# nicrie/xmca

Measured on AMD Instinct MI355X. Metric: MCA solve+rotate throughput (ms_per_step = solve+rotate wall-clock, ms); rule_n surrogates/s in `rule_n`, higher is better.
Workload: dtype f64; 1 GPU; C2: synthetic EOF T=2920 x N=10000 float64 (generator A), solve() + rotate(n_rot=10, power=1); parallelism=replicas x1 (solve/rotate do not shard); rule_n run-sharded x1

## Files before the change

xmca_amd/build.py:

```python
import os
import shutil
import subprocess
import sys

HERE = os.path.dirname(os.path.abspath(__file__))
CSRC = os.path.join(HERE, "csrc")
REPO = os.path.dirname(HERE)
LIB = os.path.join(HERE, "libxmca_hip.so")
SOURCES = ["xmca_hip.cpp"]
HEADERS = ["chol64.h", "cholesky.h", "comm.h", "common.h", "fft.h", "gemm.h", "jacobi.h", "jacobi_kernels.h", "kernels.h", "rotate.h", "solver.h", "theta.h", "tridiag.h", "tridiag_vec.h"]
ARCH = "gfx950"


def _hipcc():
    for cand in (os.environ.get("HIPCC"), shutil.which("hipcc"), "/opt/rocm/bin/hipcc"):
        if cand and os.path.exists(cand):
            return cand
    raise RuntimeError("hipcc not found (set HIPCC)")


def needs_build():
    if not os.path.exists(LIB):
        return True
    t = os.path.getmtime(LIB)
    deps = [os.path.join(CSRC, f) for f in SOURCES + HEADERS] + [os.path.join(REPO, "include", "xmca_hip.h")]
    return any(os.path.getmtime(d) > t for d in deps)


def build(force=False, verbose=True):
    if not force and not needs_build():
        return LIB
    cmd = [_hipcc(), "-x", "hip", "--offload-arch=" + ARCH, "-O3", "-std=c++17", "-fPIC", "-shared",
           "-Wall", "-Wno-unused-function", "-Wno-unused-variable", "-Wno-unused-but-set-variable",
           "-I", os.path.join(REPO, "include")]
    cmd += os.environ.get("XMCA_EXTRA_CXXFLAGS", "").split()
    cmd += [os.path.join(CSRC, s) for s in SOURCES]
    cmd += ["-ldl", "-o", LIB + ".tmp"]
    if verbose:
        print(" ".join(cmd), flush=True)
    subprocess.run(cmd, check=True)
    os.replace(LIB + ".tmp", LIB)
    return LIB

# ... 5 lines not shown
```

xmca_amd/csrc/cholesky.h:

```cpp
#pragma once
#include <hip/hip_runtime.h>

#include <cmath>
#include <cstring>

#include "common.h"
#include "gemm.h"
#include "kernels.h"
#include "chol64.h"

namespace xmca {

constexpr int CHOL_NB = C64;

__global__ void chol_zero_lower_kernel(double* __restrict__ Gr, double* __restrict__ Gi, int64_t ld, int n, const double* __restrict__ Dr,
                                       const double* __restrict__ Di) {
  const int64_t total = (int64_t)n * n;
  for (int64_t i = (int64_t)blockIdx.x * blockDim.x + threadIdx.x; i < total; i += (int64_t)gridDim.x * blockDim.x) {
    const int r = (int)(i / n), c = (int)(i % n);
    if (r > c) {
      Gr[(int64_t)r * ld + c] = 0.0;
      if (Gi) Gi[(int64_t)r * ld + c] = 0.0;
    } else if ((r >> 6) == (c >> 6)) {
      const int64_t o = (int64_t)(r >> 6) * 4096 + (r & 63) * 64 + (c & 63);
// ... 3 lines not shown
  }
}

__global__ void chol_shift_diag_kernel(double* __restrict__ Gr, int64_t ld, int n, double delta) {
  const int i = blockIdx.x * blockDim.x + threadIdx.x;
  if (i < n) Gr[(int64_t)i * ld + i] += delta;
}

__global__ void chol_max_diag_kernel(const double* __restrict__ Gr, int64_t ld, int n, unsigned long long* __restrict__ out) {
  double mx = 0.0;
  for (int i = blockIdx.x * blockDim.x + threadIdx.x; i < n; i += gridDim.x * blockDim.x) mx = fmax(mx, Gr[(int64_t)i * ld + i]);
  for (int o = 32; o > 0; o >>= 1) mx = fmax(mx, __shfl_xor(mx, o));
  if ((threadIdx.x & 63) == 0 && mx > 0.0) atomicMax(out, (unsigned long long)__double_as_longlong(mx));
}

__global__ void chol_minmax_diag_kernel(const double* __restrict__ Gr, int64_t ld, int n, unsigned long long* __restrict__ out) {
  double mx = 0.0, mn = HUGE_VAL;
  for (int i = blockIdx.x * blockDim.x + threadIdx.x; i < n; i += gridDim.x * blockDim.x) {
    const double v = Gr[(int64_t)i * ld + i];
    mx = fmax(mx, v);
    mn = fmin(mn, v);
  }
  for (int o = 32; o > 0; o >>= 1) { mx = fmax(mx, __shfl_xor(mx, o)); mn = fmin(mn, __shfl_xor(mn, o)); }
  if ((threadIdx.x & 63) == 0) {
    if (mx > 0.0) atomicMax(out, (unsigned long long)__double_as_longlong(mx));
    if (mn >= 0.0) atomicMin(out + 1, (unsigned long long)__double_as_longlong(mn));
  }
}

template <typename TI>
void cgemm(hipStream_t st, GemmWorkspace& ws, const TI* Ar, const TI* Ai, int64_t lda, bool a_kfast, bool conjA, const TI* Br,
           const TI* Bi, int64_t ldb, bool b_nfast, bool conjB, double* Cr, double* Ci, int64_t ldc, int M, int N, int K,
           double alpha, const double* row_scale, const double* col_scale, bool herm, double beta0 = 0.0,
           const GemmTileList* tiles = nullptr, int plan_rows = 0) {
  GemmOpts o;
  o.tiles = tiles;
  o.plan_rows = plan_rows;
  o.a_kfast = a_kfast;
  o.b_nfast = b_nfast;
  o.row_scale = row_scale;
  o.col_scale = col_scale;
  o.upper_only = herm;
  const double sa = conjA ? -1.0 : 1.0, sb = conjB ? -1.0 : 1.0;
  o.alpha = alpha; o.beta = beta0; o.mirror = herm ? 1 : 0;
  gemm<TI, double>(st, ws, Ar, lda, Br, ldb, Cr, ldc, M, N, K, o);
  if (Ai && Bi) {
    o.alpha = -sa * sb * alpha; o.beta = 1.0;
    gemm<TI, double>(st, ws, Ai, lda, Bi, ldb, Cr, ldc, M, N, K, o);
  }
  if (!Ci) return;
  o.mirror = herm ? -1 : 0;
  bool first = true;
  if (Bi) {
    o.alpha = sb * alpha; o.beta = beta0;
    gemm<TI, double>(st, ws, Ar, lda, Bi, ldb, Ci, ldc, M, N, K, o);
    first = false;
  }
  if (Ai) {
    o.alpha = sa * alpha; o.beta = first ? beta0 : 1.0;
    gemm<TI, double>(st, ws, Ai, lda, Br, ldb, Ci, ldc, M, N, K, o);
    first = false;
  }
  if (first && beta0 == 0.0) XMCA_HIP(hipMemsetAsync(Ci, 0, sizeof(double) * (size_t)M * ldc, st));
}

template <bool CPLX>
static void chol64_launch_panel(hipStream_t st, double* Gr, double* Gi, int64_t ld, int k0, int nb, int rest, double* Dr, double* Di, int* fail) {
  XMCA_HIP(hipFuncSetAttribute(reinterpret_cast<const void*>(chol64_panel_kernel<CPLX>), hipFuncAttributeMaxDynamicSharedMemorySize, (int)C64Lds<CPLX>::bytes()));
// ... 56 lines not shown
```

xmca_amd/csrc/gemm.h:

```cpp
#pragma once
#include <algorithm>
#include <cmath>
#include <memory>
#include <type_traits>
#include <vector>

#include "common.h"

namespace xmca {

typedef double d4_t __attribute__((ext_vector_type(4)));
typedef float f4_t __attribute__((ext_vector_type(4)));
typedef double d2_t __attribute__((ext_vector_type(2)));
typedef float f2_t __attribute__((ext_vector_type(2)));

template <typename T>
struct Mfma;
template <>
struct Mfma<double> {
  using acc_t = d4_t;
  using vec_t = d2_t;
  using frag_t = d2_t;
  static __device__ __forceinline__ acc_t mma(double a, double b, acc_t c) {
    return __builtin_amdgcn_mfma_f64_16x16x4f64(a, b, c, 0, 0, 0);
  }
  static __device__ __forceinline__ int row(int lane, int r) { return (lane >> 4) + 4 * r; }
};
template <>
struct Mfma<float> {
  using acc_t = f4_t;
  using vec_t = f4_t;
  using frag_t = f2_t;
  static __device__ __forceinline__ acc_t mma(float a, float b, acc_t c) {
    return __builtin_amdgcn_mfma_f32_16x16x4f32(a, b, c, 0, 0, 0);
  }
  static __device__ __forceinline__ int row(int lane, int r) { return (lane >> 4) * 4 + r; }
};

constexpr int GEMM_BM = 128, GEMM_BN = 128, GEMM_THREADS = 256;
constexpr int GEMM_STAGE_BYTES = 16384;
constexpr int GEMM_FLUSH_PRODUCTS = 512;
constexpr int GEMM_SLICE_PRODUCTS = 16384;
template <typename T>
struct GemmK {
  static constexpr int E = (int)sizeof(T);
  static constexpr int CE = 16 / E;
  static constexpr int BK = 128 / E;
  static constexpr int NPH = BK / 8;
};

template <typename TI, typename TO>
struct GemmParams {
  const TI* A;
  const TI* B;
  TO* C;
  int M, N, K;
  int64_t lda, ldb, ldc;
  double alpha, beta;
  const double* row_scale;
  const double* col_scale;
  int upper_only;
  int mirror;
  int k_chunk;
  int splits;
  int n_tiles;
  int n_wg;
  const int* tile_map;
  const int* tile_k;
  int vec_a, vec_b;
  double* slabs;
  int* counters;
};

template <typename TI, bool KFAST>
struct GemmOperand {
  static constexpr int E = GemmK<TI>::E, CE = GemmK<TI>::CE, BK = GemmK<TI>::BK;
  using frag_t = typename Mfma<TI>::frag_t;
  static __device__ __forceinline__ void where(int o, int& r, int& k) {
    if constexpr (KFAST) {
      r = o >> 7;
      k = (((o >> 4) & 7) ^ ((r >> 1) & 7)) * CE;
    } else {
      k = o / (128 * E);
      int c = (o % (128 * E)) >> 4;
      if constexpr (E == 4) c ^= ((k >> 1) & 1) << 3;
      r = c * CE;
    }
  }
  static __device__ __forceinline__ uint32_t voff(int lane, int jpar, int64_t ld) {
    if constexpr (KFAST) return (uint32_t)((lane >> 3) * ld * E + (((lane & 7) ^ (((lane >> 4) + 4 * jpar) & 7)) << 4));
    else if constexpr (E == 8) return (uint32_t)(lane * 16);
    else return (uint32_t)((lane >> 5) * ld * E + (((lane & 31) ^ (jpar << 3)) << 4));
  }
  static __device__ __forceinline__ uint32_t soff(int wave, int j, int64_t ld) {
    const int q = 4 * wave + j;
    return (uint32_t)((KFAST ? 8 : (E == 8 ? 1 : 2)) * q * ld * E);
  }
  static __device__ __forceinline__ uint32_t remaining(int R, int row0, int K, int k0, int64_t ld) {
    const int64_t n = KFAST ? ((int64_t)(R - 1 - row0) * ld + (K - k0)) * E : ((int64_t)(K - 1 - k0) * ld + (R - row0)) * E;
    return n > 0xffffffffll ? 0xffffffffu : (uint32_t)n;
  }
  static __device__ __forceinline__ int frag_base(int w0, int lane) {
    const int i = lane & 15, kk = lane >> 4;
    if constexpr (KFAST) {
// ... 38 lines not shown
  l = h ^ m;
  return;
#endif
  const f2_t x[4] = {f2_t{x0[0], x0[1]}, f2_t{x0[2], x0[3]}, f2_t{x1[0], x1[1]}, f2_t{x1[2], x1[3]}};
#pragma unroll
  for (int q = 0; q < 4; ++q) {
    const unsigned int hp = __builtin_bit_cast(unsigned int, __builtin_convertvector(x[q], bf16x2_t));
    h[q] = hp;
    const f2_t r = x[q] - f2_t{__uint_as_float(hp << 16), __uint_as_float(hp & 0xffff0000u)};
    const unsigned int mp = __builtin_bit_cast(unsigned int, __builtin_convertvector(r, bf16x2_t));
    m[q] = mp;
    const f2_t t = r - f2_t{__uint_as_float(mp << 16), __uint_as_float(mp & 0xffff0000u)};
    l[q] = __builtin_bit_cast(unsigned int, __builtin_convertvector(t, bf16x2_t));
  }
}

template <typename TI, typename TO, bool A_KFAST, bool B_NFAST, bool WIDE, bool X3 = false>
__global__ __launch_bounds__(GEMM_THREADS, 2) void gemm_kernel(GemmParams<TI, TO> p) {
  static_assert(!X3 || (std::is_same<TI, float>::value && A_KFAST && WIDE), "X3: float32, A contiguous along the contraction");
  using M_ = Mfma<TI>;
  using acc_t = typename M_::acc_t;
  using vec_t = typename M_::vec_t;
  using frag_t = typename M_::frag_t;
  using OA = GemmOperand<TI, A_KFAST>;
  using OB = GemmOperand<TI, !B_NFAST>;
  constexpr int CE = GemmK<TI>::CE, BK = GemmK<TI>::BK, NPH = GemmK<TI>::NPH, E = GemmK<TI>::E, SB = GEMM_STAGE_BYTES;
  __shared__ __attribute__((aligned(1024))) char smem[4 * SB];

  int L;
  {
    const int b = blockIdx.x, q = p.n_wg / 8, r = p.n_wg % 8, xcd = b % 8, idx = b / 8;
    L = (xcd < r ? xcd * (q + 1) : r * (q + 1) + (xcd - r) * q) + idx;
  }
  const int split = L / p.n_tiles, tile = L % p.n_tiles;
  const int packed = p.tile_map[tile];
  const int bm = packed >> 16, bn = packed & 0xffff;
  const int bm0 = bm * GEMM_BM, bn0 = bn * GEMM_BN;
  int kbeg, kend;
  if (p.tile_k) {
    const int kb = p.tile_k[2 * tile], ke = p.tile_k[2 * tile + 1];
    const int kc = ((ke - kb + GemmK<TI>::BK * p.splits - 1) / (GemmK<TI>::BK * p.splits)) * GemmK<TI>::BK;
    kbeg = kb + split * kc;
    kend = max(kbeg, min(ke, kbeg + kc));
  } else {
    kbeg = split * p.k_chunk;
    kend = min(p.K, kbeg + p.k_chunk);
  }

  const int wave = __builtin_amdgcn_readfirstlane((int)threadIdx.x >> 6);
  int lane = gemm_lane_id();
  const int wm = (wave >> 1) * 64, wn = (wave & 1) * 64;

  acc_t acc[X3 ? 1 : 4][X3 ? 1 : 4];
  acc_t wide[(WIDE && !X3) ? 4 : 1][(WIDE && !X3) ? 4 : 1];
  f16v_t acc3[X3 ? 2 : 1][X3 ? 2 : 1], wide3[X3 ? 2 : 1][X3 ? 2 : 1];
  if constexpr (X3) {
#pragma unroll
    for (int i = 0; i < 2; ++i)
#pragma unroll
      for (int j = 0; j < 2; ++j)
#pragma unroll
        for (int g = 0; g < 16; ++g) { acc3[i][j][g] = 0.f; wide3[i][j][g] = 0.f; }
  } else {
#pragma unroll
    for (int i = 0; i < 4; ++i)
#pragma unroll
      for (int j = 0; j < 4; ++j) {
        acc[i][j] = acc_t{0, 0, 0, 0};
        if constexpr (WIDE) wide[i][j] = acc_t{0, 0, 0, 0};
      }
  }

  const char* tileA = reinterpret_cast<const char*>(A_KFAST ? p.A + (int64_t)bm0 * p.lda : p.A + bm0);
  const char* tileB = reinterpret_cast<const char*>(B_NFAST ? p.B + bn0 : p.B + (int64_t)bn0 * p.ldb);
  const int64_t kstepA = (A_KFAST ? 1 : p.lda) * E, kstepB = (B_NFAST ? p.ldb : 1) * E;
  uint32_t va[2], vb[2];
#pragma unroll
  for (int jp = 0; jp < 2; ++jp) {
    va[jp] = OA::voff(lane, jp, p.lda);
    vb[jp] = OB::voff(lane, jp, p.ldb);
// ... 186 lines not shown
  for (int kt = nfull; kt < nkt; ++kt) {
    __syncthreads();
    stage_slow(kbeg + kt * BK, 0, tid);
    __syncthreads();
    if constexpr (X3) {
#pragma unroll
      for (int q = 0; q < 2; ++q) {
        read_frags3(smem, q);
        split3();
        mma3();
      }
    } else {
#pragma unroll
      for (int q = 0; q < NPH; ++q) {
        read_frags(smem, q, af[0], bf[0]);
        mfmas(af[0], bf[0]);
      }
    }
    flush(kt);
  }

  d2_t tot[32];
#pragma unroll
  for (int r = 0; r < 64; ++r) {
    double v;
    if constexpr (X3) v = (double)acc3[r >> 5][(r >> 4) & 1][r & 15] + (double)wide3[r >> 5][(r >> 4) & 1][r & 15];
    else {
      v = (double)acc[r >> 4][(r >> 2) & 3][r & 3];
      if constexpr (WIDE) v += (double)wide[r >> 4][(r >> 2) & 3][r & 3];
    }
    tot[r >> 1][r & 1] = v;
  }

  if (p.splits > 1) {
    double* __restrict__ mine = p.slabs + ((size_t)split * p.n_tiles + tile) * (size_t)(GEMM_BM * GEMM_BN);
#if defined(__HIP_DEVICE_COMPILE__)
    {
      const __amdgpu_buffer_rsrc_t rs = __builtin_amdgcn_make_buffer_rsrc(mine, 0, GEMM_BM * GEMM_BN * 8, 0x00020000);
#pragma unroll
      for (int h = 0; h < 32; ++h)
        __builtin_amdgcn_raw_buffer_store_b128(__builtin_bit_cast(u4_t, tot[h]), rs, tid * 16, h * 4096,  16);
    }
#endif
    asm volatile("s_waitcnt vmcnt(0)" ::: "memory");
    __syncthreads();
    int* flag = reinterpret_cast<int*>(smem);
    if (tid == 0) {
      const int ticket = __hip_atomic_fetch_add(p.counters + tile, 1, __ATOMIC_RELAXED, __HIP_MEMORY_SCOPE_AGENT);
      const int last = ticket == p.splits - 1;
      if (last) {
        __builtin_amdgcn_fence(__ATOMIC_ACQUIRE, "agent");
        __hip_atomic_store(p.counters + tile, 0, __ATOMIC_RELAXED, __HIP_MEMORY_SCOPE_AGENT);
      }
      *flag = last;
    }
    __syncthreads();
    if (*flag == 0) return;
#pragma unroll
    for (int h = 0; h < 32; ++h) tot[h] = d2_t{0, 0};
    for (int z = 0; z < p.splits; ++z) {
      const d2_t* __restrict__ sl = reinterpret_cast<const d2_t*>(p.slabs + ((size_t)z * p.n_tiles + tile) * (size_t)(GEMM_BM * GEMM_BN));
#pragma unroll
      for (int h0 = 0; h0 < 32; h0 += 8) {
#pragma unroll
        for (int h = h0; h < h0 + 8; ++h) tot[h] += sl[h * GEMM_THREADS + tid];
        asm volatile("" ::: "memory");
      }
    }
  }

  const bool offdiag = (bm != bn);
  TO* __restrict__ C = p.C;
#pragma unroll
  for (int r = 0; r < 64; ++r) {
    int rin, cin;
    if constexpr (X3) {
      const int g = r & 15;
      rin = 32 * (r >> 5) + (g & 3) + 8 * (g >> 2) + 4 * (lane >> 5);
      cin = 32 * ((r >> 4) & 1) + (lane & 31);
    } else {
      rin = OA::index(r >> 4, M_::row(lane, r & 3));
      cin = OB::index((r >> 2) & 3, lane & 15);
    }
    const int row = bm0 + wm + rin, col = bn0 + wn + cin;
    const bool sym_diag = p.mirror > 0 && !offdiag;
    if (row < p.M && col < p.N && !(sym_diag && col < row)) {
      double v = tot[r >> 1][r & 1] * p.alpha;
      if (p.row_scale) v *= p.row_scale[row];
      if (p.col_scale) v *= p.col_scale[col];
      const int64_t o = (int64_t)row * p.ldc + col;
      if (p.beta != 0.0) v += p.beta * (double)C[o];
      C[o] = (TO)v;
      if ((p.mirror != 0 && offdiag) || (sym_diag && col > row)) C[(int64_t)col * p.ldc + row] = (TO)(p.mirror > 0 ? v : -v);
    }
  }
}

struct GemmTileList {
  DevBuf<int> map;
  DevBuf<int> krange;
  int n = 0;
  int klen = 0;
  void upload(hipStream_t st, const std::vector<int>& tiles, const std::vector<int>& kr) {
    n = (int)tiles.size();
    klen = 0;
    for (int t = 0; t < n; ++t) klen = std::max(klen, kr[2 * t + 1] - kr[2 * t]);
    if (n == 0) return;
    XMCA_HIP(hipMemcpyAsync(map.ensure(tiles.size()), tiles.data(), sizeof(int) * tiles.size(), hipMemcpyHostToDevice, st));
    XMCA_HIP(hipMemcpyAsync(krange.ensure(kr.size()), kr.data(), sizeof(int) * kr.size(), hipMemcpyHostToDevice, st));
    XMCA_HIP(hipStreamSynchronize(st));
  }
};

struct GemmOpts {
  bool a_kfast = true;
  bool b_nfast = true;
  double alpha = 1.0, beta = 0.0;
  const double* row_scale = nullptr;
  const double* col_scale = nullptr;
  bool upper_only = false;
  int mirror = 0;
  int force_splits = 0;
  int plan_rows = 0;
  const GemmTileList* tiles = nullptr;
  hipEvent_t ev_begin = nullptr, ev_end = nullptr;
};

struct GemmWorkspace {
  DevBuf<double> slabs;
  DevBuf<int> counters;
  size_t counters_ready = 0;
  struct Map { int tm, tn, upper; DevBuf<int> dev; int n; };
  std::vector<std::unique_ptr<Map>> maps;
  int n_cus = 0;

  const Map& tile_map(hipStream_t st, int tm, int tn, bool upper) {
    for (auto& m : maps)
      if (m->tm == tm && m->tn == tn && m->upper == (int)upper) return *m;
    constexpr int G = 8;
    std::vector<int> order;
    for (int si = 0; si < tm; si += G)
      for (int sj = upper ? si : 0; sj < tn; sj += G)
        for (int i = si; i < std::min(si + G, tm); ++i)
          for (int j = sj; j < std::min(sj + G, tn); ++j)
            if (!upper || j >= i) order.push_back((i << 16) | j);
    auto m = std::make_unique<Map>();
    m->tm = tm; m->tn = tn; m->upper = upper; m->n = (int)order.size();
    XMCA_HIP(hipMemcpyAsync(m->dev.ensure(order.size()), order.data(), sizeof(int) * order.size(), hipMemcpyHostToDevice, st));
    XMCA_HIP(hipStreamSynchronize(st));
    maps.push_back(std::move(m));
    return *maps.back();
  }
  int* tickets(hipStream_t st, size_t n) {
    if (n > counters_ready) {
      const size_t want = std::max<size_t>(n, 4096);
      int* c = counters.ensure(want);
      XMCA_HIP(hipMemsetAsync(c, 0, sizeof(int) * counters.cap, st));
      counters_ready = counters.cap;
    }
    return counters.get();
  }
  int cus() {
    if (n_cus == 0) {
      int dev = 0, n = 256;
      (void)hipGetDevice(&dev);
      (void)hipDeviceGetAttribute(&n, hipDeviceAttributeMultiprocessorCount, dev);
      n_cus = n > 0 ? n : 256;
    }
    return n_cus;
  }
};

static inline bool gemm_x3_enabled() {
  static const bool on = [] { const char* e = std::getenv("XMCA_GEMM_BF16X3"); return !(e && e[0] == '0'); }();
  return on;
}

template <typename TI, typename TO, bool WIDE>
static void launch_gemm_variant(hipStream_t st, const GemmParams<TI, TO>& p, bool a_kfast, bool b_nfast) {
  dim3 grid(p.n_wg), block(GEMM_THREADS);
  if constexpr (std::is_same<TI, float>::value) {
    if (a_kfast && gemm_x3_enabled()) {
      if (b_nfast) hipLaunchKernelGGL((gemm_kernel<TI, TO, true, true, WIDE, true>), grid, block, 0, st, p);
      else hipLaunchKernelGGL((gemm_kernel<TI, TO, true, false, WIDE, true>), grid, block, 0, st, p);
      XMCA_HIP(hipGetLastError());
      return;
    }
  }
  if (a_kfast && b_nfast) hipLaunchKernelGGL((gemm_kernel<TI, TO, true, true, WIDE>), grid, block, 0, st, p);
  else if (a_kfast && !b_nfast) hipLaunchKernelGGL((gemm_kernel<TI, TO, true, false, WIDE>), grid, block, 0, st, p);
  else if (!a_kfast && b_nfast) hipLaunchKernelGGL((gemm_kernel<TI, TO, false, true, WIDE>), grid, block, 0, st, p);
  else hipLaunchKernelGGL((gemm_kernel<TI, TO, false, false, WIDE>), grid, block, 0, st, p);
  XMCA_HIP(hipGetLastError());
}

static inline int gemm_choose_splits(int64_t tiles, int nkt, int n_cus) {
  const int max_s = std::min(std::max(nkt / 4, 1), 128);
  int best_s = 1;
  double best = 1e300;
  for (int s = 1; s <= max_s; ++s) {
    const double q = (double)tiles * s / (2.0 * n_cus);
    const double fl = std::floor(q), phi = q - fl;
    const double rounds = fl * 1.73 + (phi < 1e-9 ? 0.0 : (phi <= 0.5 ? 1.0 : 1.73));
    const double cost = ((double)nkt / s + 8.0) * rounds * (1.0 + 0.005 * s) + (s > 1 ? (double)s : 0.0);
    if (cost < best) { best = cost; best_s = s; }
  }
  return best_s;
}

template <typename TI, typename TO>
void gemm(hipStream_t st, GemmWorkspace& ws, const TI* A, int64_t lda, const TI* B, int64_t ldb, TO* C, int64_t ldc, int M,
          int N, int K, const GemmOpts& o) {
  if (M <= 0 || N <= 0) return;
  XMCA_CHECK(!o.upper_only || M == N, XMCA_ERR_INVALID, "gemm: upper_only needs a square result");
  constexpr int BK = GemmK<TI>::BK, CE = GemmK<TI>::CE;
  const int tm = ceil_div(M, GEMM_BM), tn = ceil_div(N, GEMM_BN);
  constexpr bool WIDE = std::is_same<TI, float>::value;
  const GemmTileList* list = o.tiles;
  XMCA_CHECK(!list || (!o.upper_only && o.mirror == 0 && !WIDE), XMCA_ERR_INVALID, "gemm: tile lists are plain float64 products");
  if (list && list->n == 0) return;
  const int64_t tiles = list ? list->n : o.upper_only ? (int64_t)tm * (tm + 1) / 2 : (int64_t)tm * tn;
  const int klen = list ? list->klen : K;
  const int nkt = ceil_div(klen, BK);
  const int64_t tiles_plan = (o.plan_rows > 0 && !list && !o.upper_only) ? (int64_t)ceil_div(o.plan_rows, GEMM_BM) * tn : tiles;
  int splits = o.force_splits > 0 ? o.force_splits : gemm_choose_splits(tiles_plan, nkt, ws.cus());
  if (WIDE) splits = std::max(splits, ceil_div(K, GEMM_SLICE_PRODUCTS));
  const int* map_dev = nullptr;
  if (list) {
    map_dev = list->map.get();
  } else {
    const GemmWorkspace::Map& map = ws.tile_map(st, tm, tn, o.upper_only);
    XMCA_CHECK(map.n == tiles && tm < 65536 && tn < 65536, XMCA_ERR_INVALID, "gemm: tile map mismatch");
    map_dev = map.dev.get();
  }
  const int vec_a = lda * (int64_t)sizeof(TI) * 128 < ((int64_t)1 << 32) && reinterpret_cast<uintptr_t>(A) % sizeof(TI) == 0;
  const int vec_b = ldb * (int64_t)sizeof(TI) * 128 < ((int64_t)1 << 32) && reinterpret_cast<uintptr_t>(B) % sizeof(TI) == 0;
  int k_chunk = klen > 0 ? klen : 1;
  if (splits > 1) {
    k_chunk = ceil_div(nkt, splits) * BK;
    if (WIDE) k_chunk = std::min(k_chunk, GEMM_SLICE_PRODUCTS);
    splits = ceil_div(klen, k_chunk);
  }
  if (splits < 1 || klen <= 0) splits = 1;
  XMCA_CHECK(tiles * splits < (int64_t)1 << 31, XMCA_ERR_INVALID, "gemm: too many workgroups");
  double* slabs = nullptr;
  int* counters = nullptr;
  if (splits > 1) {
    slabs = ws.slabs.ensure((size_t)splits * tiles * GEMM_BM * GEMM_BN);
    counters = ws.tickets(st, (size_t)tiles);
  }
  GemmParams<TI, TO> p{A, B, C, M, N, K, lda, ldb, ldc, o.alpha, o.beta, o.row_scale, o.col_scale, o.upper_only ? 1 : 0, o.mirror,
                       k_chunk, splits, (int)tiles, (int)(tiles * splits), map_dev, list ? list->krange.get() : nullptr, vec_a, vec_b,
                       slabs, counters};
  if (o.ev_begin) XMCA_HIP(hipEventRecord(o.ev_begin, st));
  launch_gemm_variant<TI, TO, WIDE>(st, p, o.a_kfast, o.b_nfast);
  if (o.ev_end) XMCA_HIP(hipEventRecord(o.ev_end, st));
}

}
```

xmca_amd/csrc/tridiag_vec.h:

```cpp
#pragma once
#include "cholesky.h"
#include "tridiag.h"

namespace xmca {

__device__ __forceinline__ double trd_lane_value(double v, int u) {
  const int lo = __builtin_amdgcn_readlane(__double2loint(v), u), hi = __builtin_amdgcn_readlane(__double2hiint(v), u);
  return __hiloint2double(hi, lo);
}

__global__ __launch_bounds__(128) void trd_twisted_kernel(const double* __restrict__ d, const double* __restrict__ e, int n, int nev,
                                                         const double* __restrict__ lam, double* __restrict__ W, double* __restrict__ Yt,
                                                         int64_t ldy) {
  __shared__ double nrm_sh[2][64];
  __shared__ int idx_sh[2][64];
  const int lane = threadIdx.x & 63, half = threadIdx.x >> 6;
  const int k = blockIdx.x * 64 + lane;
  const bool live = k < nev;
  const int kk = live ? k : nev - 1;
  const double l = lam[kk];
  if (n == 1) { if (live && half == 0) Yt[k] = 1.0; return; }
  constexpr int B = 32;
  double emax = 0.0;
  for (int i = lane; i < n - 1; i += 64) emax = fmax(emax, fabs(e[i]));
// ... 382 lines not shown
}

inline bool trd_eigenvectors(hipStream_t st, TrdWorkspace& ws, TrdVecWorkspace& vw, GemmWorkspace& gws, const TrdParams& P, bool cplx,
                             double* Zr, double* Zi, int64_t ldz) {
  const int n = P.n;
  const int64_t ldv = P.ld;
  constexpr int SBK = TRD_SBK;
  const int64_t ld = ((int64_t)n + 15) & ~(int64_t)15;
  const size_t plane = (size_t)n * ld;
  double* Yr = vw.Y[0].ensure(plane);
  double* Yi = cplx ? vw.Y[1].ensure(plane) : nullptr;
  double* Wr = vw.Wk[0].ensure(plane);
  double* Wi = cplx ? vw.Wk[1].ensure(plane) : nullptr;
  hipLaunchKernelGGL(trd_twisted_kernel, dim3(ceil_div(n, 64)), dim3(128), 0, st, P.d, P.e, n, n, vw.lam_asc.get(), Wr, Yr, ld);
  XMCA_HIP(hipGetLastError());
  if (cplx) XMCA_HIP(hipMemsetAsync(Yi, 0, sizeof(double) * plane, st));
  const int nref = n - 1;
  if (nref > 0) {
    XMCA_CHECK(vw.prepared, XMCA_ERR_STATE, "trd_eigenvectors: trd_wy_prepare has not run");
    vw.prepared = false;
    if (!vw.joined) XMCA_HIP(hipStreamWaitEvent(st, vw.ev_join, 0));
    vw.joined = true;
    const double* TVr = vw.TV[0].get();
    const double* TVi = cplx ? vw.TV[1].get() : nullptr;
    double* sm = vw.small.ensure(2 * (size_t)SBK * ld);
    double* Xr = sm; double* Xi = cplx ? Xr + (size_t)SBK * ld : nullptr;
    for (int j0 = ((nref - 1) / SBK) * SBK; j0 >= 0; j0 -= SBK) {
      const int nb = std::min(SBK, nref - j0);
      const int i0 = j0 + 1, mb = n - i0;
      const int64_t vo = (int64_t)j0 * ldv + i0;
      double* Zr0 = Yr + (int64_t)i0 * ld;
      double* Zi0 = cplx ? Yi + (int64_t)i0 * ld : nullptr;
      cgemm<double>(st, gws, TVr + vo, cplx ? TVi + vo : nullptr, ldv, true, false, Zr0, Zi0, ld, true, false, Xr, Xi, ld, nb, n, mb, 1.0, nullptr,
                    nullptr, false);
      cgemm<double>(st, gws, P.Vr + vo, cplx ? P.Vi + vo : nullptr, ldv, false, false, Xr, Xi, ld, true, false, Zr0, Zi0, ld, mb, n, nb, -1.0,
                    nullptr, nullptr, false, 1.0);
    }
  }
  XMCA_HIP(hipGetLastError());
  double* Sr = vw.S[0].ensure(plane);
  double* Si = cplx ? vw.S[1].ensure(plane) : nullptr;
  vw.orth.ensure(2);
  vw.ns_steps = 0;
  for (int round = 0; round < 3; ++round) {
    cgemm<double>(st, gws, Yr, Yi, ld, false, true, Yr, Yi, ld, true, false, Sr, Si, ld, n, n, n, 1.0, nullptr, nullptr, true);
    XMCA_HIP(hipMemsetAsync(vw.orth.get(), 0, sizeof(unsigned long long) * 2, st));
    hipLaunchKernelGGL(trd_orth_kernel, dim3(std::min(n, 1024)), dim3(256), 0, st, Sr, Si, n, ld, vw.orth.get());
    hipLaunchKernelGGL(trd_ns_matrix_kernel, dim3(n), dim3(256), 0, st, Sr, Si, n, ld, 1, Wr, Wi);
    cgemm<double>(st, gws, Wr, Wi, ld, true, false, Yr, Yi, ld, false, true, Zr, Zi, ldz, n, n, n, 1.0, nullptr, nullptr, false);
    XMCA_HIP(hipGetLastError());
    unsigned long long bits = 0;
    XMCA_HIP(hipMemcpyAsync(&bits, vw.orth.get(), sizeof(bits), hipMemcpyDeviceToHost, st));
    XMCA_HIP(hipStreamSynchronize(st));
    double off;
    std::memcpy(&off, &bits, sizeof(off));
    if (round == 0) vw.last_orth = off;
    if (!(off <= 0.3)) return false;
    if (off <= 1e-6) {
      ++vw.ns_steps;
      return true;
    }
    hipLaunchKernelGGL(trd_ns_matrix_kernel, dim3(n), dim3(256), 0, st, Sr, Si, n, ld, 0, Wr, Wi);
    cgemm<double>(st, gws, Yr, Yi, ld, true, false, Wr, Wi, ld, true, false, Sr, Si, ld, n, n, n, 1.0, nullptr, nullptr, false);
    XMCA_HIP(hipMemcpyAsync(Yr, Sr, sizeof(double) * plane, hipMemcpyDeviceToDevice, st));
    if (cplx) XMCA_HIP(hipMemcpyAsync(Yi, Si, sizeof(double) * plane, hipMemcpyDeviceToDevice, st));
    ++vw.ns_steps;
  }
  return false;
}

inline bool trd_eigenvectors_partial(hipStream_t st, TrdVecWorkspace& vw, GemmWorkspace& gws, const TrdParams& P, bool cplx, int kp, int n_out,
                                     double* Zr, double* Zi, int64_t ldz) {
  const int n = P.n;
  const int64_t ldv = P.ld;
  constexpr int SBK = TRD_SBK;
  const int64_t ld = ((int64_t)kp + 15) & ~(int64_t)15;
  const size_t plane = (size_t)n * ld;
  double* Yr = vw.Y[0].ensure(plane);
  double* Yi = cplx ? vw.Y[1].ensure(plane) : nullptr;
  double* Wr = vw.Wk[0].ensure(plane);
  double* Wi = cplx ? vw.Wk[1].ensure(plane) : nullptr;
  XMCA_HIP(hipMemsetAsync(Yr, 0, sizeof(double) * plane, st));
  XMCA_HIP(hipMemsetAsync(Wr, 0, sizeof(double) * plane, st));
  if (cplx) XMCA_HIP(hipMemsetAsync(Yi, 0, sizeof(double) * plane, st));
  if (cplx) XMCA_HIP(hipMemsetAsync(Wi, 0, sizeof(double) * plane, st));
  hipLaunchKernelGGL(trd_twisted_kernel, dim3(ceil_div(kp, 64)), dim3(128), 0, st, P.d, P.e, n, kp, vw.lam_asc.get() + (n - kp), Wr, Yr, ld);
  XMCA_HIP(hipGetLastError());
  const int nref = n - 1;
  if (nref > 0) {
    XMCA_CHECK(vw.prepared, XMCA_ERR_STATE, "trd_eigenvectors_partial: trd_wy_prepare has not run");
    vw.prepared = false;
    if (!vw.joined) XMCA_HIP(hipStreamWaitEvent(st, vw.ev_join, 0));
    vw.joined = true;
    const double* TVr = vw.TV[0].get();
    const double* TVi = cplx ? vw.TV[1].get() : nullptr;
    double* sm = vw.small.ensure(2 * (size_t)SBK * ld);
    double* Xr = sm; double* Xi = cplx ? Xr + (size_t)SBK * ld : nullptr;
    for (int j0 = ((nref - 1) / SBK) * SBK; j0 >= 0; j0 -= SBK) {
      const int nb = std::min(SBK, nref - j0);
      const int i0 = j0 + 1, mb = n - i0;
      const int64_t vo = (int64_t)j0 * ldv + i0;
      double* Zr0 = Yr + (int64_t)i0 * ld;
      double* Zi0 = cplx ? Yi + (int64_t)i0 * ld : nullptr;
      cgemm<double>(st, gws, TVr + vo, cplx ? TVi + vo : nullptr, ldv, true, false, Zr0, Zi0, ld, true, false, Xr, Xi, ld, nb, kp, mb, 1.0, nullptr,
                    nullptr, false);
      cgemm<double>(st, gws, P.Vr + vo, cplx ? P.Vi + vo : nullptr, ldv, false, false, Xr, Xi, ld, true, false, Zr0, Zi0, ld, mb, kp, nb, -1.0,
                    nullptr, nullptr, false, 1.0);
    }
  }
  XMCA_HIP(hipGetLastError());
  const size_t small_plane = (size_t)kp * ld;
  double* Sr = vw.S[0].ensure(2 * small_plane);
  double* Si = cplx ? vw.S[1].ensure(2 * small_plane) : nullptr;
  double* Cr = Sr + small_plane;
  double* Ci = cplx ? Si + small_plane : nullptr;
  vw.orth.ensure(2);
  vw.ns_steps = 0;
  for (int round = 0; round < 3; ++round) {
    cgemm<double>(st, gws, Yr, Yi, ld, false, true, Yr, Yi, ld, true, false, Sr, Si, ld, kp, kp, n, 1.0, nullptr, nullptr, true);
    XMCA_HIP(hipMemsetAsync(vw.orth.get(), 0, sizeof(unsigned long long) * 2, st));
    hipLaunchKernelGGL(trd_orth_kernel, dim3(std::min(kp, 1024)), dim3(256), 0, st, Sr, Si, kp, ld, vw.orth.get());
    hipLaunchKernelGGL(trd_ns_matrix_kernel, dim3(kp), dim3(256), 0, st, Sr, Si, kp, ld, 1, Cr, Ci);
    cgemm<double>(st, gws, Cr, Ci, ld, true, false, Yr, Yi, ld, false, true, Zr, Zi, ldz, n_out, n, kp, 1.0, nullptr, nullptr, false);
    XMCA_HIP(hipGetLastError());
    unsigned long long bits = 0;
    XMCA_HIP(hipMemcpyAsync(&bits, vw.orth.get(), sizeof(bits), hipMemcpyDeviceToHost, st));
    XMCA_HIP(hipStreamSynchronize(st));
    double off;
    std::memcpy(&off, &bits, sizeof(off));
    if (round == 0) vw.last_orth = off;
    if (!(off <= 0.3)) return false;
    if (off <= 1e-6) {
      ++vw.ns_steps;
      return true;
    }
    hipLaunchKernelGGL(trd_ns_matrix_kernel, dim3(kp), dim3(256), 0, st, Sr, Si, kp, ld, 0, Cr, Ci);
    cgemm<double>(st, gws, Yr, Yi, ld, true, false, Cr, Ci, ld, true, false, Wr, Wi, ld, n, kp, kp, 1.0, nullptr, nullptr, false);
    XMCA_HIP(hipMemcpyAsync(Yr, Wr, sizeof(double) * plane, hipMemcpyDeviceToDevice, st));
    if (cplx) XMCA_HIP(hipMemcpyAsync(Yi, Wi, sizeof(double) * plane, hipMemcpyDeviceToDevice, st));
    ++vw.ns_steps;
  }
  return false;
}

}
```

Baseline: 37.29 solve+rotate/s.

## Add two-class split-K work planning to balance GEMM tail across CUs

Adds a planner that assigns tiles to two classes with different split-K factors, so the last wave of workgroups fills the CUs instead of leaving a partial round. The kernel reads a precomputed per-workgroup work list with explicit k-ranges and slab indices, and the list is cached per shape. This is enabled for the tridiagonal eigenvector back-transform and Newton-Schulz GEMMs. In exchange it adds an extra indirection, more slab reduction traffic for the long class, and a host sync the first time each plan is built.

Result: no change. 37.48 solve+rotate/s, median of 6 (+0.5%).

```diff
diff --git a/xmca_amd/build.py b/xmca_amd/build.py
--- a/xmca_amd/build.py
+++ b/xmca_amd/build.py
@@ -8,7 +8,7 @@
 REPO = os.path.dirname(HERE)
 LIB = os.path.join(HERE, "libxmca_hip.so")
 SOURCES = ["xmca_hip.cpp"]
-HEADERS = ["chol64.h", "cholesky.h", "comm.h", "common.h", "fft.h", "gemm.h", "jacobi.h", "jacobi_kernels.h", "kernels.h", "rotate.h", "solver.h", "theta.h", "tridiag.h", "tridiag_vec.h"]
+HEADERS = ["chol64.h", "cholesky.h", "comm.h", "common.h", "fft.h", "gemm.h", "gemm_plan.h", "jacobi.h", "jacobi_kernels.h", "kernels.h", "rotate.h", "solver.h", "theta.h", "tridiag.h", "tridiag_vec.h"]
 ARCH = "gfx950"
 
 
diff --git a/xmca_amd/csrc/cholesky.h b/xmca_amd/csrc/cholesky.h
--- a/xmca_amd/csrc/cholesky.h
+++ b/xmca_amd/csrc/cholesky.h
@@ -59,8 +59,9 @@
 void cgemm(hipStream_t st, GemmWorkspace& ws, const TI* Ar, const TI* Ai, int64_t lda, bool a_kfast, bool conjA, const TI* Br,
            const TI* Bi, int64_t ldb, bool b_nfast, bool conjB, double* Cr, double* Ci, int64_t ldc, int M, int N, int K,
            double alpha, const double* row_scale, const double* col_scale, bool herm, double beta0 = 0.0,
-           const GemmTileList* tiles = nullptr, int plan_rows = 0) {
+           const GemmTileList* tiles = nullptr, int plan_rows = 0, bool balance = false) {
   GemmOpts o;
+  o.balance = balance;
   o.tiles = tiles;
   o.plan_rows = plan_rows;
   o.a_kfast = a_kfast;
diff --git a/xmca_amd/csrc/gemm.h b/xmca_amd/csrc/gemm.h
--- a/xmca_amd/csrc/gemm.h
+++ b/xmca_amd/csrc/gemm.h
@@ -6,6 +6,7 @@
 #include <vector>
 
 #include "common.h"
+#include "gemm_plan.h"
 
 namespace xmca {
 
@@ -70,6 +71,7 @@
   int vec_a, vec_b;
   double* slabs;
   int* counters;
+  const GemmWork* work;
 };
 
 template <typename TI, bool KFAST>
@@ -174,20 +176,29 @@
     const int b = blockIdx.x, q = p.n_wg / 8, r = p.n_wg % 8, xcd = b % 8, idx = b / 8;
     L = (xcd < r ? xcd * (q + 1) : r * (q + 1) + (xcd - r) * q) + idx;
   }
-  const int split = L / p.n_tiles, tile = L % p.n_tiles;
+  int split, tile, nsl, slab_stride, slab_base;
+  int kbeg, kend;
+  if (std::is_same<TI, double>::value && p.work) {
+    const GemmWork w = p.work[L];
+    tile = w.tile; split = w.slice; nsl = w.slices;
+    kbeg = w.kbeg; kend = w.kend;
+    slab_stride = 1; slab_base = w.slab;
+  } else {
+    split = L / p.n_tiles; tile = L % p.n_tiles; nsl = p.splits;
+    slab_stride = p.n_tiles; slab_base = tile;
+    if (p.tile_k) {
+      const int kb = p.tile_k[2 * tile], ke = p.tile_k[2 * tile + 1];
+      const int kc = ((ke - kb + GemmK<TI>::BK * p.splits - 1) / (GemmK<TI>::BK * p.splits)) * GemmK<TI>::BK;
+      kbeg = kb + split * kc;
+      kend = max(kbeg, min(ke, kbeg + kc));
+    } else {
+      kbeg = split * p.k_chunk;
+      kend = min(p.K, kbeg + p.k_chunk);
+    }
+  }
   const int packed = p.tile_map[tile];
   const int bm = packed >> 16, bn = packed & 0xffff;
   const int bm0 = bm * GEMM_BM, bn0 = bn * GEMM_BN;
-  int kbeg, kend;
-  if (p.tile_k) {
-    const int kb = p.tile_k[2 * tile], ke = p.tile_k[2 * tile + 1];
-    const int kc = ((ke - kb + GemmK<TI>::BK * p.splits - 1) / (GemmK<TI>::BK * p.splits)) * GemmK<TI>::BK;
-    kbeg = kb + split * kc;
-    kend = max(kbeg, min(ke, kbeg + kc));
-  } else {
-    kbeg = split * p.k_chunk;
-    kend = min(p.K, kbeg + p.k_chunk);
-  }
 
   const int wave = __builtin_amdgcn_readfirstlane((int)threadIdx.x >> 6);
   int lane = gemm_lane_id();
@@ -440,8 +451,8 @@
     tot[r >> 1][r & 1] = v;
   }
 
-  if (p.splits > 1) {
-    double* __restrict__ mine = p.slabs + ((size_t)split * p.n_tiles + tile) * (size_t)(GEMM_BM * GEMM_BN);
+  if (nsl > 1) {
+    double* __restrict__ mine = p.slabs + ((size_t)split * slab_stride + slab_base) * (size_t)(GEMM_BM * GEMM_BN);
 #if defined(__HIP_DEVICE_COMPILE__)
     {
       const __amdgpu_buffer_rsrc_t rs = __builtin_amdgcn_make_buffer_rsrc(mine, 0, GEMM_BM * GEMM_BN * 8, 0x00020000);
@@ -455,7 +466,7 @@
     int* flag = reinterpret_cast<int*>(smem);
     if (tid == 0) {
       const int ticket = __hip_atomic_fetch_add(p.counters + tile, 1, __ATOMIC_RELAXED, __HIP_MEMORY_SCOPE_AGENT);
-      const int last = ticket == p.splits - 1;
+      const int last = ticket == nsl - 1;
       if (last) {
         __builtin_amdgcn_fence(__ATOMIC_ACQUIRE, "agent");
         __hip_atomic_store(p.counters + tile, 0, __ATOMIC_RELAXED, __HIP_MEMORY_SCOPE_AGENT);
@@ -466,8 +477,8 @@
     if (*flag == 0) return;
 #pragma unroll
     for (int h = 0; h < 32; ++h) tot[h] = d2_t{0, 0};
-    for (int z = 0; z < p.splits; ++z) {
-      const d2_t* __restrict__ sl = reinterpret_cast<const d2_t*>(p.slabs + ((size_t)z * p.n_tiles + tile) * (size_t)(GEMM_BM * GEMM_BN));
+    for (int z = 0; z < nsl; ++z) {
+      const d2_t* __restrict__ sl = reinterpret_cast<const d2_t*>(p.slabs + ((size_t)z * slab_stride + slab_base) * (size_t)(GEMM_BM * GEMM_BN));
 #pragma unroll
       for (int h0 = 0; h0 < 32; h0 += 8) {
 #pragma unroll
@@ -530,6 +541,7 @@
   int mirror = 0;
   int force_splits = 0;
   int plan_rows = 0;
+  bool balance = false;
   const GemmTileList* tiles = nullptr;
   hipEvent_t ev_begin = nullptr, ev_end = nullptr;
 };
@@ -559,6 +571,29 @@
     maps.push_back(std::move(m));
     return *maps.back();
   }
+  struct PlanKey { int64_t tiles; int nkt, cus; GemmPlan plan; };
+  std::vector<PlanKey> plans;
+  GemmPlan plan(int64_t tiles, int nkt, int n_cus) {
+    for (auto& k : plans)
+      if (k.tiles == tiles && k.nkt == nkt && k.cus == n_cus) return k.plan;
+    plans.push_back(PlanKey{tiles, nkt, n_cus, gemm_plan(tiles, nkt, n_cus)});
+    return plans.back().plan;
+  }
+  struct Work { int64_t tiles, n_a; int K, bk, s_a, s_b; DevBuf<GemmWork> dev; int n_wg; int64_t n_slabs; };
+  std::vector<std::unique_ptr<Work>> works;
+  const Work& work(hipStream_t st, int64_t tiles, int K, int bk, const GemmPlan& pl) {
+    for (auto& w : works)
+      if (w->tiles == tiles && w->K == K && w->bk == bk && w->n_a == pl.n_a && w->s_a == pl.s_a && w->s_b == pl.s_b) return *w;
+    std::vector<GemmWork> list;
+    auto w = std::make_unique<Work>();
+    w->tiles = tiles; w->n_a = pl.n_a; w->K = K; w->bk = bk; w->s_a = pl.s_a; w->s_b = pl.s_b;
+    w->n_slabs = gemm_build_work(pl, tiles, K, bk, list);
+    w->n_wg = (int)list.size();
+    XMCA_HIP(hipMemcpyAsync(w->dev.ensure(list.size()), list.data(), sizeof(GemmWork) * list.size(), hipMemcpyHostToDevice, st));
+    XMCA_HIP(hipStreamSynchronize(st));
+    works.push_back(std::move(w));
+    return *works.back();
+  }
   int* tickets(hipStream_t st, size_t n) {
     if (n > counters_ready) {
       const size_t want = std::max<size_t>(n, 4096);
@@ -602,18 +637,14 @@
   XMCA_HIP(hipGetLastError());
 }
 
-static inline int gemm_choose_splits(int64_t tiles, int nkt, int n_cus) {
-  const int max_s = std::min(std::max(nkt / 4, 1), 128);
-  int best_s = 1;
-  double best = 1e300;
-  for (int s = 1; s <= max_s; ++s) {
-    const double q = (double)tiles * s / (2.0 * n_cus);
-    const double fl = std::floor(q), phi = q - fl;
-    const double rounds = fl * 1.73 + (phi < 1e-9 ? 0.0 : (phi <= 0.5 ? 1.0 : 1.73));
-    const double cost = ((double)nkt / s + 8.0) * rounds * (1.0 + 0.005 * s) + (s > 1 ? (double)s : 0.0);
-    if (cost < best) { best = cost; best_s = s; }
-  }
-  return best_s;
+static inline int gemm_plan_cus(int device_cus) {
+  const char* e = std::getenv("XMCA_GEMM_CUS");
+  const int n = e ? std::atoi(e) : 0;
+  return n > 0 ? n : device_cus;
+}
+static inline bool gemm_balance_enabled() {
+  const char* e = std::getenv("XMCA_GEMM_BALANCE");
+  return !(e && e[0] == '0');
 }
 
 template <typename TI, typename TO>
@@ -631,8 +662,19 @@
   const int klen = list ? list->klen : K;
   const int nkt = ceil_div(klen, BK);
   const int64_t tiles_plan = (o.plan_rows > 0 && !list && !o.upper_only) ? (int64_t)ceil_div(o.plan_rows, GEMM_BM) * tn : tiles;
-  int splits = o.force_splits > 0 ? o.force_splits : gemm_choose_splits(tiles_plan, nkt, ws.cus());
+  const int plan_cus = gemm_plan_cus(ws.cus());
+  int splits = o.force_splits > 0 ? o.force_splits : gemm_choose_splits(tiles_plan, nkt, plan_cus);
   if (WIDE) splits = std::max(splits, ceil_div(K, GEMM_SLICE_PRODUCTS));
+  const GemmWorkspace::Work* work = nullptr;
+  if (o.balance && !WIDE && !list && o.force_splits <= 0 && o.plan_rows <= 0 && K > 0 && gemm_balance_enabled()) {
+    const GemmPlan pl = ws.plan(tiles, nkt, plan_cus);
+    if (!pl.uniform(tiles)) {
+      work = &ws.work(st, tiles, K, BK, pl);
+      if (xmca_trace("gemm"))
+        std::fprintf(stderr, "[xmca gemm] balanced M=%d N=%d K=%d upper=%d tiles=%lld n_a=%lld s_a=%d s_b=%d wg=%d\n", M, N, K, (int)o.upper_only,
+                     (long long)tiles, (long long)pl.n_a, pl.s_a, pl.s_b, work->n_wg);
+    }
+  }
   const int* map_dev = nullptr;
   if (list) {
     map_dev = list->map.get();
@@ -653,13 +695,18 @@
   XMCA_CHECK(tiles * splits < (int64_t)1 << 31, XMCA_ERR_INVALID, "gemm: too many workgroups");
   double* slabs = nullptr;
   int* counters = nullptr;
-  if (splits > 1) {
+  if (work) {
+    if (work->n_slabs > 0) {
+      slabs = ws.slabs.ensure((size_t)work->n_slabs * GEMM_BM * GEMM_BN);
+      counters = ws.tickets(st, (size_t)tiles);
+    }
+  } else if (splits > 1) {
     slabs = ws.slabs.ensure((size_t)splits * tiles * GEMM_BM * GEMM_BN);
     counters = ws.tickets(st, (size_t)tiles);
   }
   GemmParams<TI, TO> p{A, B, C, M, N, K, lda, ldb, ldc, o.alpha, o.beta, o.row_scale, o.col_scale, o.upper_only ? 1 : 0, o.mirror,
-                       k_chunk, splits, (int)tiles, (int)(tiles * splits), map_dev, list ? list->krange.get() : nullptr, vec_a, vec_b,
-                       slabs, counters};
+                       k_chunk, splits, (int)tiles, work ? work->n_wg : (int)(tiles * splits), map_dev,
+                       list ? list->krange.get() : nullptr, vec_a, vec_b, slabs, counters, work ? work->dev.get() : nullptr};
   if (o.ev_begin) XMCA_HIP(hipEventRecord(o.ev_begin, st));
   launch_gemm_variant<TI, TO, WIDE>(st, p, o.a_kfast, o.b_nfast);
   if (o.ev_end) XMCA_HIP(hipEventRecord(o.ev_end, st));
diff --git a/xmca_amd/csrc/gemm_plan.h b/xmca_amd/csrc/gemm_plan.h
--- /dev/null
+++ b/xmca_amd/csrc/gemm_plan.h
@@ -0,0 +1,117 @@
+#pragma once
+#include <algorithm>
+#include <cmath>
+#include <cstdint>
+#include <vector>
+
+namespace xmca {
+
+constexpr double GEMM_PLAN_SHARED = 1.73;
+constexpr double GEMM_PLAN_FIXED = 8.0;
+constexpr double GEMM_PLAN_TIE = 0.005;
+constexpr int GEMM_PLAN_XCDS = 8;
+
+static inline int gemm_plan_max_splits(int nkt) { return std::min(std::max(nkt / 4, 1), 128); }
+
+static inline double gemm_uniform_cost(int64_t tiles, int nkt, int n_cus, int s) {
+  const double q = (double)tiles * s / (2.0 * n_cus);
+  const double fl = std::floor(q), phi = q - fl;
+  const double rounds = fl * GEMM_PLAN_SHARED + (phi < 1e-9 ? 0.0 : (phi <= 0.5 ? 1.0 : GEMM_PLAN_SHARED));
+  return ((double)nkt / s + GEMM_PLAN_FIXED) * rounds * (1.0 + GEMM_PLAN_TIE * s) + (s > 1 ? (double)s : 0.0);
+}
+
+static inline int gemm_choose_splits(int64_t tiles, int nkt, int n_cus) {
+  const int max_s = gemm_plan_max_splits(nkt);
+  int best_s = 1;
+  double best = 1e300;
+  for (int s = 1; s <= max_s; ++s) {
+    const double cost = gemm_uniform_cost(tiles, nkt, n_cus, s);
+    if (cost < best) { best = cost; best_s = s; }
+  }
+  return best_s;
+}
+
+struct GemmPlan {
+  int64_t n_a = 0;
+  int s_a = 1, s_b = 1;
+  double cost = 0.0;
+  bool uniform(int64_t tiles) const { return n_a >= tiles; }
+};
+
+static inline double gemm_two_class_cost(int64_t tiles, int nkt, int n_cus, int64_t n_a, int s_a, int s_b) {
+  const double slots = 2.0 * n_cus;
+  const double w_a = std::ceil((double)nkt / s_a) + GEMM_PLAN_FIXED, w_b = std::ceil((double)nkt / s_b) + GEMM_PLAN_FIXED;
+  const double n_long = (double)n_a * s_a, n_short = (double)(tiles - n_a) * s_b;
+  const double units = (double)tiles * nkt + GEMM_PLAN_FIXED * (n_long + n_short);
+  const double body = std::max(std::ceil(n_long / slots) * w_a, units / slots) * GEMM_PLAN_SHARED * (1.0 + GEMM_PLAN_TIE * s_a);
+  const double tail = w_b * (n_short <= (double)n_cus ? 1.0 : GEMM_PLAN_SHARED) * (1.0 + GEMM_PLAN_TIE * s_b);
+  return body + tail + (double)s_b;
+}
+
+static inline GemmPlan gemm_plan(int64_t tiles, int nkt, int n_cus) {
+  GemmPlan best;
+  best.n_a = tiles;
+  best.s_a = best.s_b = gemm_choose_splits(tiles, nkt, n_cus);
+  best.cost = gemm_uniform_cost(tiles, nkt, n_cus, best.s_a);
+  const int max_s = gemm_plan_max_splits(nkt);
+  const int64_t slots = 2 * (int64_t)n_cus;
+  if (tiles < 2 || max_s < 2 || tiles * best.s_a <= slots) return best;
+  for (int s_a = 1; s_a < std::min(max_s, 17); ++s_a) {
+    if ((tiles * s_a) % slots == 0) continue;
+    for (int s_b = s_a + 1; s_b <= max_s; ++s_b) {
+      double prev = 1e300;
+      for (int64_t r = (tiles * s_a - 1) / slots; r >= 1; --r) {
+        const int64_t n_a = std::min(tiles - 1, r * slots / s_a);
+        if (n_a < 1) break;
+        const double c = gemm_two_class_cost(tiles, nkt, n_cus, n_a, s_a, s_b);
+        if (c < best.cost) { best.n_a = n_a; best.s_a = s_a; best.s_b = s_b; best.cost = c; }
+        if (c > prev) break;
+        prev = c;
+      }
+    }
+  }
+  return best;
+}
+
+struct GemmWork {
+  int tile;
+  int kbeg, kend;
+  int slice;
+  int slices;
+  int slab;
+  int pad0, pad1;
+};
+
+static inline int64_t gemm_build_work(const GemmPlan& pl, int64_t tiles, int K, int bk, std::vector<GemmWork>& out) {
+  const int nkt = (K + bk - 1) / bk;
+  std::vector<int> slab0((size_t)tiles, 0);
+  int64_t n_slabs = 0;
+  for (int64_t t = 0; t < tiles; ++t) {
+    const int s = t < pl.n_a ? pl.s_a : pl.s_b;
+    slab0[(size_t)t] = (int)n_slabs;
+    if (s > 1) n_slabs += s;
+  }
+  auto make = [&](std::vector<GemmWork>& cls, int64_t t0, int64_t t1, int s) {
+    for (int z = 0; z < s; ++z) {
+      const int kt0 = z * (nkt / s) + std::min(z, nkt % s), len = nkt / s + (z < nkt % s ? 1 : 0);
+      for (int64_t t = t0; t < t1; ++t)
+        cls.push_back(GemmWork{(int)t, kt0 * bk, std::min(K, (kt0 + len) * bk), z, s, slab0[(size_t)t], 0, 0});
+    }
+  };
+  std::vector<GemmWork> lng, sht;
+  make(lng, 0, pl.n_a, pl.s_a);
+  make(sht, pl.n_a, tiles, pl.s_b);
+  const int64_t nl = (int64_t)lng.size(), n = nl + (int64_t)sht.size();
+  out.clear();
+  out.reserve((size_t)n);
+  int64_t il = 0, is = 0;
+  for (int x = 0; x < GEMM_PLAN_XCDS; ++x) {
+    const int64_t len = n / GEMM_PLAN_XCDS + (x < n % GEMM_PLAN_XCDS ? 1 : 0);
+    const int64_t ll = nl / GEMM_PLAN_XCDS + (x < nl % GEMM_PLAN_XCDS ? 1 : 0);
+    for (int64_t i = 0; i < ll; ++i) out.push_back(lng[(size_t)il++]);
+    for (int64_t i = 0; i < len - ll; ++i) out.push_back(sht[(size_t)is++]);
+  }
+  return n_slabs;
+}
+
+}
diff --git a/xmca_amd/csrc/tridiag_vec.h b/xmca_amd/csrc/tridiag_vec.h
--- a/xmca_amd/csrc/tridiag_vec.h
+++ b/xmca_amd/csrc/tridiag_vec.h
@@ -438,9 +438,9 @@
       double* Zr0 = Yr + (int64_t)i0 * ld;
       double* Zi0 = cplx ? Yi + (int64_t)i0 * ld : nullptr;
       cgemm<double>(st, gws, TVr + vo, cplx ? TVi + vo : nullptr, ldv, true, false, Zr0, Zi0, ld, true, false, Xr, Xi, ld, nb, n, mb, 1.0, nullptr,
-                    nullptr, false);
+                    nullptr, false, 0.0, nullptr, 0,  true);
       cgemm<double>(st, gws, P.Vr + vo, cplx ? P.Vi + vo : nullptr, ldv, false, false, Xr, Xi, ld, true, false, Zr0, Zi0, ld, mb, n, nb, -1.0,
-                    nullptr, nullptr, false, 1.0);
+                    nullptr, nullptr, false, 1.0, nullptr, 0,  true);
     }
   }
   XMCA_HIP(hipGetLastError());
@@ -449,11 +449,11 @@
   vw.orth.ensure(2);
   vw.ns_steps = 0;
   for (int round = 0; round < 3; ++round) {
-    cgemm<double>(st, gws, Yr, Yi, ld, false, true, Yr, Yi, ld, true, false, Sr, Si, ld, n, n, n, 1.0, nullptr, nullptr, true);
+    cgemm<double>(st, gws, Yr, Yi, ld, false, true, Yr, Yi, ld, true, false, Sr, Si, ld, n, n, n, 1.0, nullptr, nullptr, true, 0.0, nullptr, 0,  true);
     XMCA_HIP(hipMemsetAsync(vw.orth.get(), 0, sizeof(unsigned long long) * 2, st));
     hipLaunchKernelGGL(trd_orth_kernel, dim3(std::min(n, 1024)), dim3(256), 0, st, Sr, Si, n, ld, vw.orth.get());
     hipLaunchKernelGGL(trd_ns_matrix_kernel, dim3(n), dim3(256), 0, st, Sr, Si, n, ld, 1, Wr, Wi);
-    cgemm<double>(st, gws, Wr, Wi, ld, true, false, Yr, Yi, ld, false, true, Zr, Zi, ldz, n, n, n, 1.0, nullptr, nullptr, false);
+    cgemm<double>(st, gws, Wr, Wi, ld, true, false, Yr, Yi, ld, false, true, Zr, Zi, ldz, n, n, n, 1.0, nullptr, nullptr, false, 0.0, nullptr, 0,  true);
     XMCA_HIP(hipGetLastError());
     unsigned long long bits = 0;
     XMCA_HIP(hipMemcpyAsync(&bits, vw.orth.get(), sizeof(bits), hipMemcpyDeviceToHost, st));
@@ -467,7 +467,7 @@
       return true;
     }
     hipLaunchKernelGGL(trd_ns_matrix_kernel, dim3(n), dim3(256), 0, st, Sr, Si, n, ld, 0, Wr, Wi);
-    cgemm<double>(st, gws, Yr, Yi, ld, true, false, Wr, Wi, ld, true, false, Sr, Si, ld, n, n, n, 1.0, nullptr, nullptr, false);
+    cgemm<double>(st, gws, Yr, Yi, ld, true, false, Wr, Wi, ld, true, false, Sr, Si, ld, n, n, n, 1.0, nullptr, nullptr, false, 0.0, nullptr, 0,  true);
     XMCA_HIP(hipMemcpyAsync(Yr, Sr, sizeof(double) * plane, hipMemcpyDeviceToDevice, st));
     if (cplx) XMCA_HIP(hipMemcpyAsync(Yi, Si, sizeof(double) * plane, hipMemcpyDeviceToDevice, st));
     ++vw.ns_steps;
@@ -509,9 +509,9 @@
       double* Zr0 = Yr + (int64_t)i0 * ld;
       double* Zi0 = cplx ? Yi + (int64_t)i0 * ld : nullptr;
       cgemm<double>(st, gws, TVr + vo, cplx ? TVi + vo : nullptr, ldv, true, false, Zr0, Zi0, ld, true, false, Xr, Xi, ld, nb, kp, mb, 1.0, nullptr,
-                    nullptr, false);
+                    nullptr, false, 0.0, nullptr, 0,  true);
       cgemm<double>(st, gws, P.Vr + vo, cplx ? P.Vi + vo : nullptr, ldv, false, false, Xr, Xi, ld, true, false, Zr0, Zi0, ld, mb, kp, nb, -1.0,
-                    nullptr, nullptr, false, 1.0);
+                    nullptr, nullptr, false, 1.0, nullptr, 0,  true);
     }
   }
   XMCA_HIP(hipGetLastError());
@@ -523,11 +523,11 @@
   vw.orth.ensure(2);
   vw.ns_steps = 0;
   for (int round = 0; round < 3; ++round) {
-    cgemm<double>(st, gws, Yr, Yi, ld, false, true, Yr, Yi, ld, true, false, Sr, Si, ld, kp, kp, n, 1.0, nullptr, nullptr, true);
+    cgemm<double>(st, gws, Yr, Yi, ld, false, true, Yr, Yi, ld, true, false, Sr, Si, ld, kp, kp, n, 1.0, nullptr, nullptr, true, 0.0, nullptr, 0,  true);
     XMCA_HIP(hipMemsetAsync(vw.orth.get(), 0, sizeof(unsigned long long) * 2, st));
     hipLaunchKernelGGL(trd_orth_kernel, dim3(std::min(kp, 1024)), dim3(256), 0, st, Sr, Si, kp, ld, vw.orth.get());
     hipLaunchKernelGGL(trd_ns_matrix_kernel, dim3(kp), dim3(256), 0, st, Sr, Si, kp, ld, 1, Cr, Ci);
-    cgemm<double>(st, gws, Cr, Ci, ld, true, false, Yr, Yi, ld, false, true, Zr, Zi, ldz, n_out, n, kp, 1.0, nullptr, nullptr, false);
+    cgemm<double>(st, gws, Cr, Ci, ld, true, false, Yr, Yi, ld, false, true, Zr, Zi, ldz, n_out, n, kp, 1.0, nullptr, nullptr, false, 0.0, nullptr, 0,  true);
     XMCA_HIP(hipGetLastError());
     unsigned long long bits = 0;
     XMCA_HIP(hipMemcpyAsync(&bits, vw.orth.get(), sizeof(bits), hipMemcpyDeviceToHost, st));
@@ -541,7 +541,7 @@
       return true;
     }
     hipLaunchKernelGGL(trd_ns_matrix_kernel, dim3(kp), dim3(256), 0, st, Sr, Si, kp, ld, 0, Cr, Ci);
-    cgemm<double>(st, gws, Yr, Yi, ld, true, false, Cr, Ci, ld, true, false, Wr, Wi, ld, n, kp, kp, 1.0, nullptr, nullptr, false);
+    cgemm<double>(st, gws, Yr, Yi, ld, true, false, Cr, Ci, ld, true, false, Wr, Wi, ld, n, kp, kp, 1.0, nullptr, nullptr, false, 0.0, nullptr, 0,  true);
     XMCA_HIP(hipMemcpyAsync(Yr, Wr, sizeof(double) * plane, hipMemcpyDeviceToDevice, st));
     if (cplx) XMCA_HIP(hipMemcpyAsync(Yi, Wi, sizeof(double) * plane, hipMemcpyDeviceToDevice, st));
     ++vw.ns_steps;
```
